# dpwe/audfprint

Hardware: NVIDIA H100
Metric: audio_seconds_fingerprinted_per_sec (higher is better)
Workload: dtype f64

## Files before the change

### audfprint_b200/csrc/afp_stft.cu

```cuda
#include <math.h>
#include <algorithm>
#include "afp_fft.cuh"
#include "afp_internal.cuh"
#include "afp_tma.cuh"

namespace {

constexpr int FT = AFP_FRAMES_PER_TILE;
constexpr int XS = 17;
constexpr int XF = 16 * XS;
constexpr int K1_THREADS = 256;
constexpr int LOGTAB = 64;
constexpr int LOGCOPIES = 8;

__device__ __forceinline__ int64_t reflect_index(int64_t j, int64_t n) {
  if (n == 1) return 0;
  const int64_t period = 2 * (n - 1);
  int64_t r = j % period;
  if (r < 0) r += period;
  return r < n ? r : period - r;
}

__device__ __forceinline__ double int_to_double(int x) {
  return __hiloint2double(0x43380000 + (x >> 31), x) - 6755399441055744.0;
}

__device__ __noinline__ double half_log_quarter_slow(double v) { return 0.5 * log(0.25 * v); }
__device__ __forceinline__ bool is_special(double v) {
  return (unsigned)(__double2hiint(v) - 0x00100000) >= 0x7fe00000u;
}

__constant__ double k1_log_c64[8] = {0.5 / 7.0, -0.5 / 6.0, 0.5 / 5.0, -0.5 / 4.0,
                                     0.5 / 3.0, -0.5 / 2.0, 0.5,       0.34657359027997264};

__device__ __forceinline__ double half_log_quarter(double v, const double2* s_logtab_lane) {
  const int hi = __double2hiint(v);
  const int lo = __double2loint(v);
  const double m = __hiloint2double((hi & 0x000fffff) | 0x3ff00000, lo);
  const double2 ct = s_logtab_lane[((hi >> 14) & (LOGTAB - 1)) * LOGCOPIES];
  const double r = fma(m, ct.x, -1.0);
  double p = k1_log_c64[0];
  p = fma(p, r, k1_log_c64[1]);
  p = fma(p, r, k1_log_c64[2]);
  p = fma(p, r, k1_log_c64[3]);
  p = fma(p, r, k1_log_c64[4]);
  p = fma(p, r, k1_log_c64[5]);
  p = fma(p, r, k1_log_c64[6]);
  const double ed = int_to_double((hi >> 20) - 1025);
  return fma(ed, k1_log_c64[7], ct.y) + p * r;
}

template <typename PcmT> struct PcmTraits;
template <> struct PcmTraits<int16_t> {
  static constexpr int NBUF = 2;
};
template <> struct PcmTraits<float> {
  static constexpr int NBUF = 1;
};

template <typename R> struct K1Traits;

template <> struct K1Traits<double> {
  using R2 = double2;
  static constexpr int MIN_CTAS = 2;
  static constexpr int LOGTAB_N = LOGTAB * LOGCOPIES;
  static constexpr int HMIN_NONE = 0x7ff00000;
  __device__ static __forceinline__ void load2(const int16_t* p, double& a, double& b) {
    const uint32_t w = *reinterpret_cast<const uint32_t*>(p);
    a = int_to_double((int)(short)(w & 0xffffu));
    b = int_to_double((int)w >> 16);
  }
  __device__ static __forceinline__ void load2(const float* p, double& a, double& b) {
    const float2 w = *reinterpret_cast<const float2*>(p);
    a = (double)w.x;
    b = (double)w.y;
  }
  __device__ static __forceinline__ int hbits(double v) { return __double2hiint(v); }
  __device__ static __forceinline__ void log_pair(double ssa, double ssb, const double2* tab, double& la,
                                                  double& lb) {
    la = half_log_quarter(ssa, tab);
    lb = half_log_quarter(ssb, tab);
    if (is_special(ssa) || is_special(ssb)) {
      la = half_log_quarter_slow(ssa);
      lb = half_log_quarter_slow(ssb);
    }
  }
  __device__ static __forceinline__ double log1(double ss, const double2* tab) {
    double lg = half_log_quarter(ss, tab);
    if (is_special(ss)) lg = half_log_quarter_slow(ss);
    return lg;
  }
  __device__ static __forceinline__ double log_lower_bound(int hmin, const double2* tab) {
    const double v_lo = __hiloint2double(hmin, 0);
    return hmin >= HMIN_NONE ? INFINITY : (hmin < 0x00100000 ? -INFINITY : half_log_quarter(v_lo, tab));
  }
};

template <> struct K1Traits<float> {
  using R2 = float2;
  static constexpr int MIN_CTAS = 3;
  static constexpr int LOGTAB_N = 0;
  static constexpr int HMIN_NONE = 0x7f800000;
  __device__ static __forceinline__ void load2(const int16_t* p, float& a, float& b) {
    const uint32_t w = *reinterpret_cast<const uint32_t*>(p);
    a = (float)(short)(w & 0xffffu);
    b = (float)((int)w >> 16);
  }
  __device__ static __forceinline__ void load2(const float* p, float& a, float& b) {
    const float2 w = *reinterpret_cast<const float2*>(p);
    a = w.x;
    b = w.y;
  }
  __device__ static __forceinline__ int hbits(float v) { return __float_as_int(v); }
  __device__ static __forceinline__ void log_pair(float ssa, float ssb, const double2*, float& la, float& lb) {
    la = 0.5f * __logf(0.25f * ssa);
    lb = 0.5f * __logf(0.25f * ssb);
  }
  __device__ static __forceinline__ float log1(float ss, const double2*) { return 0.5f * __logf(0.25f * ss); }
  __device__ static __forceinline__ double log_lower_bound(int hmin, const double2*) {
    return hmin >= HMIN_NONE ? INFINITY
           : (hmin < 0x00800000 ? -INFINITY : (double)(0.5f * __logf(0.25f * __int_as_float(hmin))) - 1e-6);
  }
};

template <typename R>
struct StftArgs {
  using R2 = typename K1Traits<R>::R2;
  const void* pcm;
  const ItemDesc* items;
  const int32_t* tile_item;
  int nitems;
  int tile_begin, tile_end;
  const R* window;
  const R2* tw256;
  const R2* w512;
  const double2* logtab;
  R* logs;
  double* nyq;
  double* tile_stats;
  double* mag;
};

struct TileInfo {
  int64_t frame0;
  int64_t src;
  int64_t j0;
  int64_t nsamples;
  int nft;
  int tma;
};

template <typename PcmT>
__device__ __forceinline__ TileInfo make_tile(const PcmT* pcm, const ItemDesc& it, int tile) {
  TileInfo ti;
  const int t0 = (tile - it.tile_base) * FT;
  ti.frame0 = it.frame_base + t0;
  ti.nft = min(FT, it.nframes - t0);
  ti.j0 = (int64_t)(t0 - 1) * AFP_N_HOP;
  ti.src = it.sample_start + ti.j0;
  ti.nsamples = it.nsamples;
  constexpr int GR = 16 / (int)sizeof(PcmT);
  const int64_t run_n = (int64_t)(ti.nft + 1) * AFP_N_HOP;
  const int64_t lo = ti.j0 < 0 ? -ti.j0 : 0;
  const int64_t hi = (ti.j0 + run_n <= it.nsamples ? run_n : it.nsamples - ti.j0) & ~(int64_t)(GR - 1);
  const bool aligned = (reinterpret_cast<uintptr_t>(pcm + ti.src) & 15) == 0;
  ti.tma = (aligned && hi > lo) ? (int)((lo << 16) | (hi - lo)) : 0;
  return ti;
}

template <typename PcmT>
__device__ __forceinline__ void stage_tile(const PcmT* pcm, const TileInfo& ti, PcmT* dst, unsigned long long* bar) {
  const int nsamp = (ti.nft + 1) * AFP_N_HOP;
  const int t_first = ti.tma >> 16, t_count = ti.tma & 0xffff;
  if (t_count && threadIdx.x == 0) bulk_copy_g2s(dst + t_first, pcm + ti.src + t_first, t_count * sizeof(PcmT), bar);
  if (t_count != nsamp) {
    const PcmT* item0 = pcm + (ti.src - ti.j0);
    for (int i = threadIdx.x; i < nsamp - t_count; i += K1_THREADS) {
      const int p = i < t_first ? i : i + t_count;
      dst[p] = item0[reflect_index(ti.j0 + p, ti.nsamples)];
    }
  }
}

template <typename R, typename PcmT>
constexpr size_t k1_smem_bytes() {
  return 512 * sizeof(R) + 2 * 256 * sizeof(typename K1Traits<R>::R2) + K1Traits<R>::LOGTAB_N * sizeof(double2) +
         2 * FT * XF * sizeof(R) + 2 * 24 * sizeof(double) + 2 * sizeof(unsigned long long) +
         PcmTraits<PcmT>::NBUF * (FT + 1) * AFP_N_HOP * sizeof(PcmT);
}

template <typename R, typename PcmT, bool WRITE_MAG>
__global__ void __launch_bounds__(K1_THREADS, K1Traits<R>::MIN_CTAS)
    afp_stft_kernel(const __grid_constant__ StftArgs<R> a) {
  using Tr = K1Traits<R>;
  using R2 = typename Tr::R2;
  constexpr int NBUF = PcmTraits<PcmT>::NBUF;
  extern __shared__ __align__(16) unsigned char smem_raw[];
  R* s_win = reinterpret_cast<R*>(smem_raw);
  R2* s_tw256 = reinterpret_cast<R2*>(s_win + 512);
  R2* s_w512 = s_tw256 + 256;
  double2* s_logtab_all = reinterpret_cast<double2*>(s_w512 + 256);
  R* s_xr = reinterpret_cast<R*>(s_logtab_all + Tr::LOGTAB_N);
  R* s_xi = s_xr + FT * XF;
  double* s_red = reinterpret_cast<double*>(s_xi + FT * XF);
  unsigned long long* s_bar = reinterpret_cast<unsigned long long*>(s_red + 2 * 24);
  PcmT* s_pcm = reinterpret_cast<PcmT*>(s_bar + 2);
  constexpr int PCM_BUF = (FT + 1) * AFP_N_HOP;
  const PcmT* pcm = reinterpret_cast<const PcmT*>(a.pcm);

  const int tid = threadIdx.x;
  if (tid == 0) mbar_init<2>(s_bar);
  for (int i = tid; i < 512; i += K1_THREADS) s_win[i] = a.window[i];
  for (int i = tid; i < 256; i += K1_THREADS) {
    s_tw256[i] = a.tw256[i];
    s_w512[i] = a.w512[i];
  }
  if constexpr (Tr::LOGTAB_N > 0)
    for (int i = tid; i < Tr::LOGTAB_N; i += K1_THREADS) s_logtab_all[i] = a.logtab[i];
  __syncthreads();

  const int g = tid >> 4;
  const int r = tid & 15;
  const int lane = tid & 31;
  const double2* s_logtab = s_logtab_all + (lane & (LOGCOPIES - 1));
  const int src_lane = (lane & 16) | ((16 - r) & 15);
  uint32_t phases = 0u;

  int tile = a.tile_begin + blockIdx.x;
  if (tile >= a.tile_end) return;
  const int G = gridDim.x;
  TileInfo cur = make_tile(pcm, a.items[a.tile_item[tile]], tile);
  TileInfo nxt = cur;
  if (tile + G < a.tile_end) nxt = make_tile(pcm, a.items[a.tile_item[tile + G]], tile + G);
  int item_nn = (tile + 2 * G < a.tile_end) ? a.tile_item[tile + 2 * G] : 0;
  stage_tile(pcm, cur, s_pcm, s_bar);
  int buf = 0;
  int red = 0;

  for (; tile < a.tile_end; tile += G) {
    const int next = tile + G;
    if (NBUF == 2 && next < a.tile_end) stage_tile(pcm, nxt, s_pcm + (buf ^ 1) * PCM_BUF, s_bar + (buf ^ 1));
    ItemDesc desc_nn = a.items[item_nn];
    const int item_n3 = (tile + 3 * G < a.tile_end) ? a.tile_item[tile + 3 * G] : 0;
    if (cur.tma & 0xffff) {
      mbar_wait(s_bar + buf, (phases >> buf) & 1u);
      phases ^= 1u << buf;
    }
    if ((cur.tma & 0xffff) != (cur.nft + 1) * AFP_N_HOP) __syncthreads();

    const bool active = g < cur.nft;
    const int64_t frame = cur.frame0 + g;
    R vmax = 0, vsum = 0;
    int hmin = Tr::HMIN_NONE;
    R zr[16], zi[16];
    if (active) {
      const PcmT* fr = s_pcm + buf * PCM_BUF + g * AFP_N_HOP;
#pragma unroll
      for (int q = 0; q < 16; ++q) {
        const int i0 = 2 * (16 * q + r);
        const R2 w = *reinterpret_cast<const R2*>(s_win + i0);
        R x0, x1;
        Tr::load2(fr + i0, x0, x1);
        zr[q] = x0 * w.x;
        zi[q] = x1 * w.y;
      }
      afp_fft16(zr, zi);
      R* xr = s_xr + g * XF;
      R* xi = s_xi + g * XF;
#pragma unroll
      for (int p = 0; p < 16; ++p) {
        const R2 w = s_tw256[p * 16 + r];
        xr[p * XS + r] = zr[p] * w.x - zi[p] * w.y;
        xi[p * XS + r] = zr[p] * w.y + zi[p] * w.x;
      }
    }
    __syncwarp();
    if (active) {
      const R* xr = s_xr + g * XF + r * XS;
      const R* xi = s_xi + g * XF + r * XS;
#pragma unroll
      for (int q = 0; q < 16; ++q) {
        zr[q] = xr[q];
        zi[q] = xi[q];
      }
      afp_fft16(zr, zi);
    }
    {
      R* out = a.logs + frame * AFP_NBINS;
#pragma unroll
      for (int s = 0; s < 8; ++s) {
        R c = __shfl_sync(0xffffffffu, zr[15 - s], src_lane);
        R d = __shfl_sync(0xffffffffu, zi[15 - s], src_lane);
        if (r == 0) {
          c = zr[(16 - s) & 15];
          d = zi[(16 - s) & 15];
        }
        if (active) {
          const int k = r + 16 * s;
          const R2 w = s_w512[k];
          const R er = zr[s] + c, ei = zi[s] - d, orr = zi[s] + d, oi = c - zr[s];
          const R pr = w.x * orr - w.y * oi, pi = w.x * oi + w.y * orr;
          const R ar = er + pr, ai = ei + pi, br = er - pr, bi = ei - pi;
          const R ssa = ar * ar + ai * ai;
          const R ssb = br * br + bi * bi;
          R la, lb;
          Tr::log_pair(ssa, ssb, s_logtab, la, lb);
          out[k] = la;
          if (k != 0) out[256 - k] = lb; else a.nyq[frame] = lb;
          if (WRITE_MAG) {
            a.mag[frame * 257 + k] = sqrt(R(0.25) * ssa);
            a.mag[frame * 257 + 256 - k] = sqrt(R(0.25) * ssb);
          }
          vmax = fmax(vmax, fmax(ssa, ssb));
          hmin = min(hmin, min(Tr::hbits(ssa), Tr::hbits(ssb)));
          vsum += la + lb;
        }
      }
      if (active && r == 0) {
        const R2 w = s_w512[128];
        const R er = R(2) * zr[8], orr = R(2) * zi[8];
        const R ar = er + w.x * orr, ai = w.y * orr;
        const R ss = ar * ar + ai * ai;
        const R lg = Tr::log1(ss, s_logtab);
        out[128] = lg;
        if (WRITE_MAG) a.mag[frame * 257 + 128] = sqrt(R(0.25) * ss);
        vmax = fmax(vmax, ss);
        hmin = min(hmin, Tr::hbits(ss));
        vsum += lg;
      }
    }
    hmin = __reduce_min_sync(0xffffffffu, hmin);
    const double vmin = Tr::log_lower_bound(hmin, s_logtab);
    double dmax = vmax, dsum = vsum;
#pragma unroll
    for (int o = 16; o > 0; o >>= 1) {
      dmax = fmax(dmax, __shfl_xor_sync(0xffffffffu, dmax, o));
      dsum += __shfl_xor_sync(0xffffffffu, dsum, o);
    }
    double* const s_part = s_red + 24 * (NBUF == 2 ? buf : red);
    if (lane == 0) {
      s_part[(tid >> 5) * 3 + 0] = dmax;
      s_part[(tid >> 5) * 3 + 1] = vmin;
      s_part[(tid >> 5) * 3 + 2] = dsum;
    }
    __syncthreads();
    if (tid == 0) {
      double m = 0.0, mn = INFINITY, sm = 0.0;
#pragma unroll
      for (int w = 0; w < K1_THREADS / 32; ++w) {
        m = fmax(m, s_part[w * 3 + 0]);
        mn = fmin(mn, s_part[w * 3 + 1]);
        sm += s_part[w * 3 + 2];
      }
      a.tile_stats[(size_t)tile * 3 + 0] = 0.25 * m;
      a.tile_stats[(size_t)tile * 3 + 1] = mn;
      a.tile_stats[(size_t)tile * 3 + 2] = sm;
    }
    if (NBUF == 2) buf ^= 1; else red ^= 1;
    cur = nxt;
    if (tile + 2 * G < a.tile_end) nxt = make_tile(pcm, desc_nn, tile + 2 * G);
    item_nn = item_n3;
    if (NBUF == 1 && next < a.tile_end) stage_tile(pcm, cur, s_pcm, s_bar);
  }
}

__global__ void afp_tile_table_kernel(const ItemDesc* items, int nitems, int32_t* tile_item) {
  const int i = blockIdx.x * blockDim.x + threadIdx.x;
  if (i >= nitems) return;
  const ItemDesc it = items[i];
  const int nt = (it.nframes + FT - 1) / FT;
  for (int k = 0; k < nt; ++k) tile_item[it.tile_base + k] = i;
}

__global__ void __launch_bounds__(256) afp_stats_kernel(const ItemDesc* items, int item0, int nitems,
                                                        const double* tile_stats, ItemStats* out, int phase) {
  const int lane = threadIdx.x & 31;
  const int w = blockIdx.x * (blockDim.x >> 5) + (threadIdx.x >> 5);
  if (w >= nitems) return;
  const int item = item0 + w;
  if (phase == 1 && !out[item].floored) return;
  const ItemDesc it = items[item];
  const int ntiles = (it.nframes + FT - 1) / FT;
  double m = 0.0, mn = INFINITY, sm = 0.0;
  for (int i = lane; i < ntiles; i += 32) {
    const double* ts = tile_stats + (size_t)(it.tile_base + i) * 3;
    m = fmax(m, ts[0]);
    mn = fmin(mn, ts[1]);
    sm += ts[2];
  }
#pragma unroll
  for (int o = 16; o > 0; o >>= 1) {
    m = fmax(m, __shfl_xor_sync(0xffffffffu, m, o));
    mn = fmin(mn, __shfl_xor_sync(0xffffffffu, mn, o));
    sm += __shfl_xor_sync(0xffffffffu, sm, o);
  }
  if (lane == 0) {
    const bool allzero = !(m > 0.0);
    ItemStats st;
    st.logfloor = allzero ? 0.0 : log(sqrt(m) / 1e6);
    st.mean = (allzero || it.nframes == 0) ? 0.0 : sm / ((double)it.nframes * 257.0);
    st.allzero = allzero ? 1 : 0;
    st.floored = (phase == 0 && !allzero && mn < st.logfloor) ? 1 : 0;
    out[item] = st;
  }
}

constexpr int FS_SPLIT = 8;
template <typename R>
__global__ void __launch_bounds__(256) afp_floorsum_kernel(const ItemDesc* items, int item0, const ItemStats* stats,
                                                           const R* logs, const double* nyq,
                                                           double* tile_stats) {
  __shared__ double s_part[8];
  const int item = item0 + blockIdx.x;
  const ItemStats st = stats[item];
  if (!st.floored) return;
  const ItemDesc it = items[item];
  const int ntiles = (it.nframes + FT - 1) / FT;
  for (int k = blockIdx.y; k < ntiles; k += FS_SPLIT) {
    const int t0 = k * FT, nft = min(FT, it.nframes - t0);
    const R* L = logs + (size_t)(it.frame_base + t0) * AFP_NBINS;
    double acc = 0.0;
    for (int i = threadIdx.x; i < nft * AFP_NBINS; i += 256) acc += fmax((double)L[i], st.logfloor);
    if ((int)threadIdx.x < nft) acc += fmax(nyq[it.frame_base + t0 + threadIdx.x], st.logfloor);
#pragma unroll
    for (int o = 16; o > 0; o >>= 1) acc += __shfl_xor_sync(0xffffffffu, acc, o);
    __syncthreads();
    if ((threadIdx.x & 31) == 0) s_part[threadIdx.x >> 5] = acc;
    __syncthreads();
    if (threadIdx.x == 0) {
      double t = 0.0;
      for (int w = 0; w < 8; ++w) t += s_part[w];
      tile_stats[(size_t)(it.tile_base + k) * 3 + 2] = t;
    }
  }
}

template <typename R>
__global__ void afp_sgram_kernel(const ItemDesc* items, const ItemStats* stats, const R* logs,
                                 double pole, double* out) {
  const ItemDesc it = items[blockIdx.x];
  const ItemStats st = stats[blockIdx.x];
  const int b = threadIdx.x;
  double z = 0.0;
  for (int t = 0; t < it.nframes; ++t) {
    const size_t idx = (size_t)(it.frame_base + t) * AFP_NBINS + b;
    double x = st.allzero ? 0.0 : __dsub_rn(fmax((double)logs[idx], st.logfloor), st.mean);
    const double y = __dadd_rn(z, x);
    z = __dadd_rn(-x, __dmul_rn(pole, y));
    out[idx] = y;
  }
}

}

int afp_launch_tile_table(afp_ctx* c) {
  if (c->nitems == 0) return AFP_OK;
  afp_tile_table_kernel<<<(c->nitems + 255) / 256, 256, 0, c->stream>>>(c->d_items.as<ItemDesc>(), c->nitems,
                                                                       c->d_tile_item.as<int32_t>());
  AFP_CUDA(c, cudaGetLastError());
  c->launches++;
  return AFP_OK;
}

namespace {

template <typename R, typename PcmT, bool WRITE_MAG>
cudaError_t launch_k1(const StftArgs<R>& a, int num_sms, int64_t ntiles, cudaStream_t stream) {
  constexpr size_t smem = k1_smem_bytes<R, PcmT>();
  const int nctas = (int)std::min<int64_t>(ntiles, (int64_t)num_sms * K1Traits<R>::MIN_CTAS);
  const cudaError_t e =
      cudaFuncSetAttribute(afp_stft_kernel<R, PcmT, WRITE_MAG>, cudaFuncAttributeMaxDynamicSharedMemorySize, (int)smem);
  if (e == cudaSuccess) afp_stft_kernel<R, PcmT, WRITE_MAG><<<nctas, K1_THREADS, smem, stream>>>(a);
  return e;
}

template <typename R>
cudaError_t launch_stft(afp_ctx* c, const DevBuf& window, const DevBuf& twid, const void* pcm, int dtype,
                        double* mag_out, int64_t tile0, int64_t ntiles) {
  using R2 = typename K1Traits<R>::R2;
  StftArgs<R> a;
  a.pcm = pcm;
  a.items = c->d_items.as<ItemDesc>();
  a.tile_item = c->d_tile_item.as<int32_t>();
  a.nitems = c->nitems;
  a.tile_begin = (int)tile0;
  a.tile_end = (int)(tile0 + ntiles);
  a.window = window.as<R>() + (dtype == AFP_PCM_I16 ? AFP_N_FFT : 0);
  a.tw256 = twid.as<R2>();
  a.w512 = twid.as<R2>() + 256;
  a.logtab = c->d_twid.as<double2>() + 512;
  a.logs = c->d_logs.as<R>();
  a.nyq = c->d_nyq.as<double>();
  a.tile_stats = c->d_tile_stats.as<double>();
  a.mag = mag_out;
  const int n = c->num_sms;
  if (dtype == AFP_PCM_I16)
    return mag_out ? launch_k1<R, int16_t, true>(a, n, ntiles, c->stream)
                   : launch_k1<R, int16_t, false>(a, n, ntiles, c->stream);
  return mag_out ? launch_k1<R, float, true>(a, n, ntiles, c->stream)
                 : launch_k1<R, float, false>(a, n, ntiles, c->stream);
}

}

int afp_launch_stft(afp_ctx* c, const void* pcm, int dtype, double* mag_out, int64_t tile0, int64_t ntiles) {
  if (ntiles <= 0) return AFP_OK;
  const cudaError_t e =
      c->ap.spectrogram_fp32
          ? launch_stft<float>(c, c->d_window_f, c->d_twid_f, pcm, dtype, mag_out, tile0, ntiles)
          : launch_stft<double>(c, c->d_window, c->d_twid, pcm, dtype, mag_out, tile0, ntiles);
  AFP_CUDA(c, e);
  AFP_CUDA(c, cudaGetLastError());
  c->launches++;
  return AFP_OK;
}

int afp_launch_stats(afp_ctx* c, int item0, int nitems) {
  if (nitems <= 0) return AFP_OK;
  const ItemDesc* items = c->d_items.as<ItemDesc>();
  ItemStats* st = c->d_item_stats.as<ItemStats>();
  double* ts = c->d_tile_stats.as<double>();
  afp_stats_kernel<<<(nitems + 7) / 8, 256, 0, c->stream>>>(items, item0, nitems, ts, st, 0);
  AFP_CUDA(c, cudaGetLastError());
  if (c->ap.spectrogram_fp32)
    afp_floorsum_kernel<float><<<dim3((unsigned)nitems, FS_SPLIT), 256, 0, c->stream>>>(
        items, item0, st, c->d_logs.as<float>(), c->d_nyq.as<double>(), ts);
  else
    afp_floorsum_kernel<double><<<dim3((unsigned)nitems, FS_SPLIT), 256, 0, c->stream>>>(
        items, item0, st, c->d_logs.as<double>(), c->d_nyq.as<double>(), ts);
  AFP_CUDA(c, cudaGetLastError());
  afp_stats_kernel<<<(nitems + 7) / 8, 256, 0, c->stream>>>(items, item0, nitems, ts, st, 1);
  AFP_CUDA(c, cudaGetLastError());
  c->launches += 3;
  return AFP_OK;
}

int afp_launch_sgram(afp_ctx* c, double* sgram_out) {
  if (c->nitems == 0 || c->total_frames == 0) return AFP_OK;
  if (c->ap.spectrogram_fp32)
    afp_sgram_kernel<float><<<c->nitems, AFP_NBINS, 0, c->stream>>>(
        c->d_items.as<ItemDesc>(), c->d_item_stats.as<ItemStats>(), c->d_logs.as<float>(), c->ap.hpf_pole, sgram_out);
  else
    afp_sgram_kernel<double><<<c->nitems, AFP_NBINS, 0, c->stream>>>(
        c->d_items.as<ItemDesc>(), c->d_item_stats.as<ItemStats>(), c->d_logs.as<double>(), c->ap.hpf_pole, sgram_out);
  AFP_CUDA(c, cudaGetLastError());
  c->launches++;
  return AFP_OK;
}
```

### audfprint_b200/csrc/afp_peaks.cu

```cuda
#include <math.h>
#include "afp_internal.cuh"
#include "afp_tma.cuh"

namespace {

constexpr unsigned FULL = 0xffffffffu;
constexpr int CH = 4;
constexpr int NST = 2;
constexpr int PFB = 8;

constexpr int K2_CTAS_PER_SM = 10;
constexpr size_t K2_SMEM_BUDGET = 233472 / K2_CTAS_PER_SM - 1024;
constexpr size_t k2_static_smem(size_t rsize) {
  return sizeof(double) * AFP_GAUSS_PAD + 128  + NST * CH * AFP_NBINS * rsize +
         NST * sizeof(unsigned long long);
}
static_assert(k2_static_smem(sizeof(double)) <= K2_SMEM_BUDGET,
              "K2's shared memory would fit fewer than 10 CTAs per SM: a 1024-item batch would run in two waves");

struct PeakArgs {
  const ItemDesc* items;
  const ItemStats* stats;
  int item0;
  const void* logs;
  const double* gauss;
  double a_dec, pole;
  int maxpks;
  double* fwd_val;
  uint8_t* fwd_bin;
  uint8_t* fwd_cnt;
  uint8_t* pk_bin;
  uint8_t* pk_cnt;
  int32_t* item_scols;
  int32_t* item_npeaks;
};

__device__ __forceinline__ int bin_of(int lane, int j) { return 8 * lane + j; }
__device__ __forceinline__ int lane_of(int pos) { return pos >> 3; }
__device__ __forceinline__ int reg_of(int pos) { return pos & 7; }
__device__ __forceinline__ int gidx(int k) { return k + (k >> 3); }

__device__ __forceinline__ void bump(double (&thr)[8], const double* sE, int lane, int pos, double val) {
  const int k0 = AFP_NBINS - pos + 8 * lane;
  const uint32_t e0 = smem_u32(sE + gidx(k0)), e1 = e0 + 8;
  const int split = 8 - (k0 & 7);
#pragma unroll
  for (int j = 0; j < 8; ++j) {
    double e;
    asm volatile("ld.shared.f64 %0, [%1];" : "=d"(e) : "r"((j >= split ? e1 : e0) + 8 * j) : "memory");
    const double p = __dmul_rn(val, e);
    thr[j] = p > thr[j] ? p : thr[j];
  }
}

__device__ __forceinline__ double pick(const double (&v)[8], int j) {
  double x = v[0];
#pragma unroll
  for (int i = 1; i < 8; ++i) x = (j == i) ? v[i] : x;
  return x;
}

__device__ __forceinline__ unsigned locmax_mask(const double (&s)[8], int lane) {
  const double left = __shfl_up_sync(FULL, s[7], 1);
  const double right = __shfl_down_sync(FULL, s[0], 1);
  bool ge[9];
  ge[0] = (lane == 0) ? true : (s[0] >= left);
#pragma unroll
  for (int j = 1; j < 8; ++j) ge[j] = s[j] >= s[j - 1];
  ge[8] = (lane == 31) ? false : (right >= s[7]);
  unsigned m = 0;
#pragma unroll
  for (int j = 0; j < 8; ++j) m |= (ge[j] && !ge[j + 1]) ? (1u << j) : 0u;
  return m;
}

__device__ __forceinline__ void spread(const double (&v)[8], double (&thr)[8], const double* sE, int lane) {
#pragma unroll
  for (int j = 0; j < 8; ++j) thr[j] = 0.0;
  const unsigned m = locmax_mask(v, lane);
  unsigned lanes = __ballot_sync(FULL, m != 0);
  while (lanes) {
    const int src = __ffs(lanes) - 1;
    lanes &= lanes - 1;
    unsigned mm = __shfl_sync(FULL, m, src);
    while (mm) {
      const int j = __ffs(mm) - 1;
      mm &= mm - 1;
      const double val = __shfl_sync(FULL, pick(v, j), src);
      bump(thr, sE, lane, bin_of(src, j), val);
    }
  }
}

__device__ __forceinline__ void hpf_step(const double (&l)[8], double (&z)[8], double (&s)[8], double lf,
                                         double mean, double pole) {
#pragma unroll
  for (int j = 0; j < 8; ++j) {
    const double x = __dsub_rn(fmax(l[j], lf), mean);
    const double y = __dadd_rn(z[j], x);
    z[j] = __dadd_rn(-x, __dmul_rn(pole, y));
    s[j] = y;
  }
}

template <typename R>
struct ColRing {
  R* buf;
  unsigned long long* bar;
  const R* src;
  int T;
  int lane;

  __device__ __forceinline__ void issue(int chunk) const {
    const int c0 = chunk * CH;
    const uint32_t bytes = (uint32_t)min(CH, T - c0) * AFP_NBINS * sizeof(R);
    bulk_copy_g2s(buf + (chunk % NST) * CH * AFP_NBINS, src + (size_t)c0 * AFP_NBINS, bytes, bar + (chunk % NST));
  }
  __device__ __forceinline__ void wait(int chunk) const { mbar_wait(bar + (chunk % NST), (chunk / NST) & 1); }
  __device__ __forceinline__ void read(const R* col, double (&x)[8]) const {
    if (sizeof(R) == 8) {
      const double2* p = reinterpret_cast<const double2*>(col) + 4 * lane;
#pragma unroll
      for (int i = 0; i < 4; ++i) {
        const double2 v = p[i];
        x[2 * i] = v.x;
        x[2 * i + 1] = v.y;
      }
    } else {
      const float4* p = reinterpret_cast<const float4*>(col) + 2 * lane;
      const float4 u = p[0], v = p[1];
      x[0] = u.x; x[1] = u.y; x[2] = u.z; x[3] = u.w;
      x[4] = v.x; x[5] = v.y; x[6] = v.z; x[7] = v.w;
    }
  }
  __device__ __forceinline__ void peek(int t, double (&x)[8]) const { read(src + (size_t)t * AFP_NBINS, x); }
  __device__ __forceinline__ void load(int t, double (&x)[8]) const {
    const int chunk = t / CH;
    if (t % CH == 0) wait(chunk);
    read(buf + ((chunk % NST) * CH + t % CH) * AFP_NBINS, x);
    if (t % CH == CH - 1 || t == T - 1) {
      __syncwarp();
      if (lane == 0 && (chunk + NST) * CH < T) issue(chunk + NST);
    }
  }
};

template <typename R>
__global__ void __launch_bounds__(32) afp_peaks_kernel(PeakArgs a) {
  __shared__ __align__(16) double sE[AFP_GAUSS_PAD];
  __shared__ __align__(128) R sCol[NST * CH * AFP_NBINS];
  __shared__ unsigned long long sBar[NST];
  const int lane = threadIdx.x;
  const int item = a.item0 + blockIdx.x;
  for (int k = lane; k < AFP_GAUSS_N; k += 32) sE[gidx(k)] = a.gauss[k];

  const ItemDesc it = a.items[item];
  const ItemStats st = a.stats[item];
  const int T = it.nframes;
  const int64_t base = it.frame_base;
  const int maxpks = a.maxpks;
  if (T == 0 || st.allzero) {
    for (int t = lane; t < T; t += 32) a.pk_cnt[base + t] = 0;
    if (lane == 0) {
      a.item_scols[item] = 0;
      a.item_npeaks[item] = 0;
    }
    return;
  }
  ColRing<R> ring{sCol, sBar, reinterpret_cast<const R*>(a.logs) + base * AFP_NBINS, T, lane};
  if (lane == 0) {
    mbar_init<NST>(sBar);
    for (int c = 0; c < NST && c * CH < T; ++c) ring.issue(c);
  }
  __syncwarp();
  const double lf = st.logfloor, mean = st.mean, pole = a.pole, a_dec = a.a_dec;

  double thr[8], z[8], s[8], sn[8], l[8];

  {
    double mx[8];
#pragma unroll
    for (int j = 0; j < 8; ++j) { z[j] = 0.0; mx[j] = -INFINITY; }
    const int n0 = min(10, T);
    for (int t = 0; t < n0; ++t) {
      ring.peek(t, l);
      hpf_step(l, z, s, lf, mean, pole);
#pragma unroll
      for (int j = 0; j < 8; ++j) mx[j] = fmax(mx[j], s[j]);
    }
    spread(mx, thr, sE, lane);
  }

#pragma unroll
  for (int j = 0; j < 8; ++j) z[j] = 0.0;
  ring.load(0, l);
  hpf_step(l, z, s, lf, mean, pole);
  unsigned lm = locmax_mask(s, lane);
  for (int t = 0; t < T; ++t) {
    unsigned lmn = 0;
    if (t + 1 < T) {
      ring.load(t + 1, l);
      hpf_step(l, z, sn, lf, mean, pole);
      lmn = locmax_mask(sn, lane);
    }
    unsigned cmask = lm;
#pragma unroll
    for (int j = 0; j < 8; ++j) cmask &= (s[j] > thr[j]) ? ~0u : ~(1u << j);
    int npk = 0;
    if (__ballot_sync(FULL, cmask != 0)) {
      while (true) {
        unsigned long long bk = 0ull;
        int bj = -1;
#pragma unroll
        for (int j = 0; j < 8; ++j) {
          const unsigned long long k = (unsigned long long)__double_as_longlong(s[j]);
          if (((cmask >> j) & 1u) && k >= bk) { bk = k; bj = j; }
        }
        const unsigned hi = (unsigned)(bk >> 32), lo = (unsigned)bk;
        const unsigned mhi = __reduce_max_sync(FULL, bj >= 0 ? hi : 0u);
        const bool v1 = bj >= 0 && hi == mhi;
        const unsigned mlo = __reduce_max_sync(FULL, v1 ? lo : 0u);
        const bool v2 = v1 && lo == mlo;
        const int pos = (int)__reduce_max_sync(FULL, v2 ? (unsigned)(bin_of(lane, bj) + 1) : 0u) - 1;
        const double val = __longlong_as_double((long long)(((unsigned long long)mhi << 32) | mlo));
        if (lane == lane_of(pos)) cmask &= ~(1u << reg_of(pos));
        bump(thr, sE, lane, pos, val);
        if (lane == 0) {
          a.fwd_val[(base + t) * maxpks + npk] = val;
          a.fwd_bin[(base + t) * maxpks + npk] = (uint8_t)pos;
        }
        ++npk;
        if (npk >= maxpks || !__ballot_sync(FULL, cmask != 0)) break;
      }
    }
    if (lane == 0) a.fwd_cnt[base + t] = (uint8_t)npk;
#pragma unroll
    for (int j = 0; j < 8; ++j) thr[j] = __dmul_rn(thr[j], a_dec);
    if (t + 1 < T) {
#pragma unroll
      for (int j = 0; j < 8; ++j) s[j] = sn[j];
      lm = lmn;
    }
  }
  __syncwarp();

  spread(s, thr, sE, lane);
  int nxt_bin = -1, nxt_alive = 0;
  int scols = 0, npeaks = 0;
  auto emit = [&](int col, int bin, int alive) {
    const unsigned am = __ballot_sync(FULL, alive != 0);
    int rank = 0;
    unsigned mm = am;
    while (mm) {
      const int src = __ffs(mm) - 1;
      mm &= mm - 1;
      const int b = __shfl_sync(FULL, bin, src);
      rank += (b < bin) ? 1 : 0;
    }
    if (alive) a.pk_bin[(base + col) * maxpks + rank] = (uint8_t)bin;
    const int c = __popc(am);
    if (lane == 0) a.pk_cnt[base + col] = (uint8_t)c;
    if (c) scols = max(scols, col + 1);
    npeaks += c;
  };
  int pc[PFB], pb[PFB];
  double pv[PFB];
  const bool slot = lane < maxpks;
  auto fetch = [&](int t, int& c, double& v, int& b) {
    c = a.fwd_cnt[base + t];
    v = slot ? a.fwd_val[(base + t) * maxpks + lane] : 0.0;
    b = slot ? (int)a.fwd_bin[(base + t) * maxpks + lane] : -1;
  };
#pragma unroll
  for (int u = 0; u < PFB; ++u)
    if (T - 1 - u >= 0) fetch(T - 1 - u, pc[u], pv[u], pb[u]);
  for (int t0 = T - 1; t0 >= 0; t0 -= PFB) {
#pragma unroll
    for (int u = 0; u < PFB; ++u) {
      const int t = t0 - u;
      if (t >= 0) {
        const int n = pc[u];
        const double my_val = pv[u];
        const int my_bin = (lane < n) ? pb[u] : -1;
        if (t - PFB >= 0) fetch(t - PFB, pc[u], pv[u], pb[u]);
        int cur_alive = 0;
        for (int k = 0; k < n; ++k) {
          const double val = __shfl_sync(FULL, my_val, k);
          const int pos = __shfl_sync(FULL, my_bin, k);
          const bool ok = val >= pick(thr, reg_of(pos));
          if ((__ballot_sync(FULL, ok) >> lane_of(pos)) & 1u) {
            bump(thr, sE, lane, pos, val);
            if (lane == k) cur_alive = 1;
            if (nxt_alive && nxt_bin == pos) nxt_alive = 0;
          }
        }
#pragma unroll
        for (int j = 0; j < 8; ++j) thr[j] = __dmul_rn(a_dec, thr[j]);
        if (t + 1 < T) emit(t + 1, nxt_bin, nxt_alive);
        nxt_bin = my_bin;
        nxt_alive = cur_alive;
      }
    }
  }
  emit(0, nxt_bin, nxt_alive);
  if (lane == 0) {
    a.item_scols[item] = scols;
    a.item_npeaks[item] = npeaks;
  }
}

__global__ void __launch_bounds__(256) afp_peaks_compact_kernel(const ItemDesc* items, int shifts, int shift,
                                                                int maxpks, const uint8_t* pk_bin,
                                                                const uint8_t* pk_cnt, const int64_t* off,
                                                                int32_t* rows) {
  __shared__ int s_scan[256];
  __shared__ int s_run;
  const ItemDesc it = items[blockIdx.x * shifts + shift];
  const int tid = threadIdx.x;
  if (tid == 0) s_run = 0;
  __syncthreads();
  int32_t* out = rows + 2 * off[blockIdx.x];
  for (int t0 = 0; t0 < it.nframes; t0 += 256) {
    const int t = t0 + tid;
    const int c = (t < it.nframes) ? pk_cnt[it.frame_base + t] : 0;
    s_scan[tid] = c;
    __syncthreads();
    for (int o = 1; o < 256; o <<= 1) {
      const int v = (tid >= o) ? s_scan[tid - o] : 0;
      __syncthreads();
      s_scan[tid] += v;
      __syncthreads();
    }
    const int excl = s_scan[tid] - c + s_run;
    for (int i = 0; i < c; ++i) {
      out[2 * (excl + i)] = t;
      out[2 * (excl + i) + 1] = pk_bin[(it.frame_base + t) * maxpks + i];
    }
    __syncthreads();
    if (tid == 255) s_run += s_scan[255];
    __syncthreads();
  }
}

__global__ void afp_gather_npeaks_kernel(const int32_t* item_npeaks, int nfiles, int shifts, int shift,
                                         int32_t* out) {
  const int f = blockIdx.x * blockDim.x + threadIdx.x;
  if (f < nfiles) out[f] = item_npeaks[f * shifts + shift];
}

__global__ void __launch_bounds__(256) afp_spread_kernel(const double* vec, int n, const double* tab,
                                                        const double* base, double* out) {
  extern __shared__ int s_pk[];
  __shared__ int s_n;
  if (threadIdx.x == 0) s_n = 0;
  __syncthreads();
  for (int i = threadIdx.x; i < n; i += blockDim.x) {
    const bool ge = (i == 0) ? true : (vec[i] >= vec[i - 1]);
    const bool ge_next = (i == n - 1) ? false : (vec[i + 1] >= vec[i]);
    if (ge && !ge_next) s_pk[atomicAdd(&s_n, 1)] = i;
  }
  __syncthreads();
  const int np = s_n;
  for (int i = threadIdx.x; i < n; i += blockDim.x) {
    double v = base ? base[i] : 0.0;
    for (int k = 0; k < np; ++k) {
      const int p = s_pk[k];
      v = fmax(v, __dmul_rn(vec[p], tab[i + n - p]));
    }
    out[i] = v;
  }
}

}

int afp_spread_peaks_impl(afp_ctx* c, const double* vector, int32_t n, const double* table, double width,
                          const double* base, double* out) {
  const size_t nn = (size_t)n;
  AFP_CUDA(c, c->d_tmp.reserve(sizeof(double) * (5 * nn + 8)));
  double* d_vec = c->d_tmp.as<double>();
  double* d_tab = d_vec + nn;
  double* d_base = d_tab + 2 * nn + 1;
  double* d_out = d_base + nn;
  std::vector<double> tab(2 * nn + 1);
  for (size_t j = 0; j < tab.size(); ++j) {
    const double u = ((double)j - (double)n) / width;
    tab[j] = table ? table[j] : exp(-0.5 * (u * u));
  }
  AFP_CUDA(c, cudaMemcpyAsync(d_vec, vector, sizeof(double) * nn, cudaMemcpyHostToDevice, c->stream));
  AFP_CUDA(c, cudaMemcpyAsync(d_tab, tab.data(), sizeof(double) * tab.size(), cudaMemcpyHostToDevice, c->stream));
  if (base) AFP_CUDA(c, cudaMemcpyAsync(d_base, base, sizeof(double) * nn, cudaMemcpyHostToDevice, c->stream));
  const size_t smem = sizeof(int) * nn;
  if (smem > 48 * 1024)
    AFP_CUDA(c, cudaFuncSetAttribute(afp_spread_kernel, cudaFuncAttributeMaxDynamicSharedMemorySize, (int)smem));
  afp_spread_kernel<<<1, 256, smem, c->stream>>>(d_vec, n, d_tab, base ? d_base : nullptr, d_out);
  AFP_CUDA(c, cudaGetLastError());
  c->launches++;
  AFP_CUDA(c, cudaMemcpyAsync(out, d_out, sizeof(double) * nn, cudaMemcpyDeviceToHost, c->stream));
  AFP_CUDA(c, cudaStreamSynchronize(c->stream));
  return AFP_OK;
}

int afp_launch_peaks(afp_ctx* c, int item0, int nitems) {
  if (nitems <= 0) return AFP_OK;
  PeakArgs a;
  a.items = c->d_items.as<ItemDesc>();
  a.stats = c->d_item_stats.as<ItemStats>();
  a.item0 = item0;
  a.logs = c->d_logs.p;
  a.gauss = c->d_gauss.as<double>();
  a.a_dec = c->ap.a_dec;
  a.pole = c->ap.hpf_pole;
  a.maxpks = c->ap.maxpksperframe;
  a.fwd_val = c->d_fwd_val.as<double>();
  a.fwd_bin = c->d_fwd_bin.as<uint8_t>();
  a.fwd_cnt = c->d_fwd_cnt.as<uint8_t>();
  a.pk_bin = c->d_pk_bin.as<uint8_t>();
  a.pk_cnt = c->d_pk_cnt.as<uint8_t>();
  a.item_scols = c->d_item_scols.as<int32_t>();
  a.item_npeaks = c->d_item_npeaks.as<int32_t>();
  if (!c->peaks_carveout_set) {
    AFP_CUDA(c, cudaFuncSetAttribute(afp_peaks_kernel<double>, cudaFuncAttributePreferredSharedMemoryCarveout,
                                     cudaSharedmemCarveoutMaxShared));
    AFP_CUDA(c, cudaFuncSetAttribute(afp_peaks_kernel<float>, cudaFuncAttributePreferredSharedMemoryCarveout,
                                     cudaSharedmemCarveoutMaxShared));
    c->peaks_carveout_set = true;
  }
  if (c->ap.spectrogram_fp32) afp_peaks_kernel<float><<<nitems, 32, 0, c->stream>>>(a);
  else afp_peaks_kernel<double><<<nitems, 32, 0, c->stream>>>(a);
  AFP_CUDA(c, cudaGetLastError());
  c->launches++;
  return AFP_OK;
}

int afp_compact_peaks(afp_ctx* c, int shift) {
  AFP_CUDA(c, c->d_tmp.reserve(sizeof(int32_t) * (size_t)(c->nfiles + 1)));
  AFP_CUDA(c, c->d_pk_off.reserve(sizeof(int64_t) * (size_t)(c->nfiles + 1)));
  afp_gather_npeaks_kernel<<<(c->nfiles + 255) / 256, 256, 0, c->stream>>>(
      c->d_item_npeaks.as<int32_t>(), c->nfiles, c->ap.shifts, shift, c->d_tmp.as<int32_t>());
  AFP_CUDA(c, cudaGetLastError());
  c->launches++;
  int rc = afp_launch_scan_i32_to_i64(c, c->d_tmp.as<int32_t>(), c->d_pk_off.as<int64_t>(), c->nfiles);
  if (rc) return rc;
  int64_t total = 0;
  AFP_CUDA(c, cudaMemcpyAsync(&total, c->d_pk_off.as<int64_t>() + c->nfiles, sizeof(int64_t),
                              cudaMemcpyDeviceToHost, c->stream));
  AFP_CUDA(c, cudaStreamSynchronize(c->stream));
  AFP_CUDA(c, c->d_pk_rows.reserve(sizeof(int32_t) * 2 * (size_t)(total + 1)));
  if (total > 0) {
    afp_peaks_compact_kernel<<<c->nfiles, 256, 0, c->stream>>>(
        c->d_items.as<ItemDesc>(), c->ap.shifts, shift, c->ap.maxpksperframe, c->d_pk_bin.as<uint8_t>(),
        c->d_pk_cnt.as<uint8_t>(), c->d_pk_off.as<int64_t>(), c->d_pk_rows.as<int32_t>());
    AFP_CUDA(c, cudaGetLastError());
    c->launches++;
  }
  return AFP_OK;
}
```

Before: 6.693 million.

## Interleave FFT scratch as complex pairs, replace shuffles with smem mirror, batch special-case logs

Stores the STFT transpose scratch as interleaved complex pairs instead of split real and imaginary arrays, which halves the number of shared-memory instructions per element. The mirrored-bin exchange for the real-FFT post-processing now goes through shared memory instead of warp shuffles, and all of it sits inside the active branch, guarded by partial-warp syncwarp masks. The per-element special-value checks on the log are replaced by a fast path plus one fallback recompute per thread, triggered from hmin/hmax. The exponent-to-double conversion is also simplified. The risks are extra shared-memory traffic, the reworked sync masks, and registers for the ss array.

```diff
diff --git a/audfprint_b200/csrc/afp_stft.cu b/audfprint_b200/csrc/afp_stft.cu
--- a/audfprint_b200/csrc/afp_stft.cu
+++ b/audfprint_b200/csrc/afp_stft.cu
@@ -30,8 +30,8 @@
   return (unsigned)(__double2hiint(v) - 0x00100000) >= 0x7fe00000u;
 }
 
-__constant__ double k1_log_c64[8] = {0.5 / 7.0, -0.5 / 6.0, 0.5 / 5.0, -0.5 / 4.0,
-                                     0.5 / 3.0, -0.5 / 2.0, 0.5,       0.34657359027997264};
+__constant__ double k1_log_c64[9] = {0.5 / 7.0, -0.5 / 6.0, 0.5 / 5.0, -0.5 / 4.0, 0.5 / 3.0,
+                                     -0.5 / 2.0, 0.5,       0.34657359027997264, 4503599627371521.0};
 
 __device__ __forceinline__ double half_log_quarter(double v, const double2* s_logtab_lane) {
   const int hi = __double2hiint(v);
@@ -46,7 +46,7 @@
   p = fma(p, r, k1_log_c64[4]);
   p = fma(p, r, k1_log_c64[5]);
   p = fma(p, r, k1_log_c64[6]);
-  const double ed = int_to_double((hi >> 20) - 1025);
+  const double ed = __hiloint2double(0x43300000, (unsigned)hi >> 20) - k1_log_c64[8];
   return fma(ed, k1_log_c64[7], ct.y) + p * r;
 }
 
@@ -76,6 +76,11 @@
     b = (double)w.y;
   }
   __device__ static __forceinline__ int hbits(double v) { return __double2hiint(v); }
+  __device__ static __forceinline__ double log_fast(double v, const double2* tab) { return half_log_quarter(v, tab); }
+  __device__ static __forceinline__ bool any_special(int hmin, int hmax) {
+    return hmin < 0x00100000 || hmax >= 0x7ff00000;
+  }
+  __device__ static __forceinline__ double max2(double x, double y) { return x > y ? x : y; }
   __device__ static __forceinline__ void log_pair(double ssa, double ssb, const double2* tab, double& la,
                                                   double& lb) {
     la = half_log_quarter(ssa, tab);
@@ -112,6 +117,9 @@
     b = w.y;
   }
   __device__ static __forceinline__ int hbits(float v) { return __float_as_int(v); }
+  __device__ static __forceinline__ float log_fast(float v, const double2*) { return 0.5f * __logf(0.25f * v); }
+  __device__ static __forceinline__ bool any_special(int, int) { return false; }
+  __device__ static __forceinline__ float max2(float x, float y) { return fmaxf(x, y); }
   __device__ static __forceinline__ void log_pair(float ssa, float ssb, const double2*, float& la, float& lb) {
     la = 0.5f * __logf(0.25f * ssa);
     lb = 0.5f * __logf(0.25f * ssb);
@@ -185,7 +193,7 @@
 template <typename R, typename PcmT>
 constexpr size_t k1_smem_bytes() {
   return 512 * sizeof(R) + 2 * 256 * sizeof(typename K1Traits<R>::R2) + K1Traits<R>::LOGTAB_N * sizeof(double2) +
-         2 * FT * XF * sizeof(R) + 2 * 24 * sizeof(double) + 2 * sizeof(unsigned long long) +
+         FT * XF * sizeof(typename K1Traits<R>::R2) + 2 * 24 * sizeof(double) + 2 * sizeof(unsigned long long) +
          PcmTraits<PcmT>::NBUF * (FT + 1) * AFP_N_HOP * sizeof(PcmT);
 }
 
@@ -200,9 +208,8 @@
   R2* s_tw256 = reinterpret_cast<R2*>(s_win + 512);
   R2* s_w512 = s_tw256 + 256;
   double2* s_logtab_all = reinterpret_cast<double2*>(s_w512 + 256);
-  R* s_xr = reinterpret_cast<R*>(s_logtab_all + Tr::LOGTAB_N);
-  R* s_xi = s_xr + FT * XF;
-  double* s_red = reinterpret_cast<double*>(s_xi + FT * XF);
+  R2* s_xz = reinterpret_cast<R2*>(s_logtab_all + Tr::LOGTAB_N);
+  double* s_red = reinterpret_cast<double*>(s_xz + FT * XF);
   unsigned long long* s_bar = reinterpret_cast<unsigned long long*>(s_red + 2 * 24);
   PcmT* s_pcm = reinterpret_cast<PcmT*>(s_bar + 2);
   constexpr int PCM_BUF = (FT + 1) * AFP_N_HOP;
@@ -223,7 +230,6 @@
   const int r = tid & 15;
   const int lane = tid & 31;
   const double2* s_logtab = s_logtab_all + (lane & (LOGCOPIES - 1));
-  const int src_lane = (lane & 16) | ((16 - r) & 15);
   uint32_t phases = 0u;
 
   int tile = a.tile_begin + blockIdx.x;
@@ -252,8 +258,10 @@
     const int64_t frame = cur.frame0 + g;
     R vmax = 0, vsum = 0;
     int hmin = Tr::HMIN_NONE;
-    R zr[16], zi[16];
     if (active) {
+      const unsigned amask = 2 * (tid >> 5) + 1 < cur.nft ? 0xffffffffu : 0x0000ffffu;
+      R2* const xz = s_xz + g * XF;
+      R zr[16], zi[16];
       const PcmT* fr = s_pcm + buf * PCM_BUF + g * AFP_N_HOP;
 #pragma unroll
       for (int q = 0; q < 16; ++q) {
@@ -265,67 +273,78 @@
         zi[q] = x1 * w.y;
       }
       afp_fft16(zr, zi);
-      R* xr = s_xr + g * XF;
-      R* xi = s_xi + g * XF;
 #pragma unroll
       for (int p = 0; p < 16; ++p) {
         const R2 w = s_tw256[p * 16 + r];
-        xr[p * XS + r] = zr[p] * w.x - zi[p] * w.y;
-        xi[p * XS + r] = zr[p] * w.y + zi[p] * w.x;
-      }
-    }
-    __syncwarp();
-    if (active) {
-      const R* xr = s_xr + g * XF + r * XS;
-      const R* xi = s_xi + g * XF + r * XS;
+        xz[p * XS + r] = R2{zr[p] * w.x - zi[p] * w.y, zr[p] * w.y + zi[p] * w.x};
+      }
+      __syncwarp(amask);
 #pragma unroll
       for (int q = 0; q < 16; ++q) {
-        zr[q] = xr[q];
-        zi[q] = xi[q];
+        const R2 v = xz[r * XS + q];
+        zr[q] = v.x;
+        zi[q] = v.y;
       }
       afp_fft16(zr, zi);
-    }
-    {
+      __syncwarp(amask);
+#pragma unroll
+      for (int s = 8; s < 16; ++s) xz[r + 16 * s] = R2{zr[s], zi[s]};
+      if (r == 0) xz[256] = R2{zr[0], zi[0]};
+      __syncwarp(amask);
+      const R2* const zp = xz + 256 - r;
       R* out = a.logs + frame * AFP_NBINS;
+      R ss[16];
+      int hmax = 0;
 #pragma unroll
       for (int s = 0; s < 8; ++s) {
-        R c = __shfl_sync(0xffffffffu, zr[15 - s], src_lane);
-        R d = __shfl_sync(0xffffffffu, zi[15 - s], src_lane);
-        if (r == 0) {
-          c = zr[(16 - s) & 15];
-          d = zi[(16 - s) & 15];
+        const R2 p = zp[-16 * s];
+        const R c = p.x, d = p.y;
+        const int k = r + 16 * s;
+        const R2 w = s_w512[k];
+        const R er = zr[s] + c, ei = zi[s] - d, orr = zi[s] + d, oi = c - zr[s];
+        const R pr = w.x * orr - w.y * oi, pi = w.x * oi + w.y * orr;
+        const R ar = er + pr, ai = ei + pi, br = er - pr, bi = ei - pi;
+        const R ssa = ar * ar + ai * ai;
+        const R ssb = br * br + bi * bi;
+        ss[2 * s] = ssa;
+        ss[2 * s + 1] = ssb;
+        const R la = Tr::log_fast(ssa, s_logtab), lb = Tr::log_fast(ssb, s_logtab);
+        out[k] = la;
+        if (k != 0) out[256 - k] = lb; else a.nyq[frame] = lb;
+        if (WRITE_MAG) {
+          a.mag[frame * 257 + k] = sqrt(R(0.25) * ssa);
+          a.mag[frame * 257 + 256 - k] = sqrt(R(0.25) * ssb);
         }
-        if (active) {
+        vmax = Tr::max2(vmax, Tr::max2(ssa, ssb));
+        hmin = min(hmin, min(Tr::hbits(ssa), Tr::hbits(ssb)));
+        hmax = max(hmax, max(Tr::hbits(ssa), Tr::hbits(ssb)));
+        vsum += la + lb;
+      }
+      if (Tr::any_special(hmin, hmax)) {
+        vmax = 0;
+        vsum = 0;
+#pragma unroll
+        for (int s = 0; s < 8; ++s) {
           const int k = r + 16 * s;
-          const R2 w = s_w512[k];
-          const R er = zr[s] + c, ei = zi[s] - d, orr = zi[s] + d, oi = c - zr[s];
-          const R pr = w.x * orr - w.y * oi, pi = w.x * oi + w.y * orr;
-          const R ar = er + pr, ai = ei + pi, br = er - pr, bi = ei - pi;
-          const R ssa = ar * ar + ai * ai;
-          const R ssb = br * br + bi * bi;
           R la, lb;
-          Tr::log_pair(ssa, ssb, s_logtab, la, lb);
+          Tr::log_pair(ss[2 * s], ss[2 * s + 1], s_logtab, la, lb);
           out[k] = la;
           if (k != 0) out[256 - k] = lb; else a.nyq[frame] = lb;
-          if (WRITE_MAG) {
-            a.mag[frame * 257 + k] = sqrt(R(0.25) * ssa);
-            a.mag[frame * 257 + 256 - k] = sqrt(R(0.25) * ssb);
-          }
-          vmax = fmax(vmax, fmax(ssa, ssb));
-          hmin = min(hmin, min(Tr::hbits(ssa), Tr::hbits(ssb)));
+          vmax = fmax(vmax, fmax(ss[2 * s], ss[2 * s + 1]));
           vsum += la + lb;
         }
       }
-      if (active && r == 0) {
+      if (r == 0) {
         const R2 w = s_w512[128];
-        const R er = R(2) * zr[8], orr = R(2) * zi[8];
+        const R2 z = xz[128];
+        const R er = R(2) * z.x, orr = R(2) * z.y;
         const R ar = er + w.x * orr, ai = w.y * orr;
-        const R ss = ar * ar + ai * ai;
-        const R lg = Tr::log1(ss, s_logtab);
+        const R s128 = ar * ar + ai * ai;
+        const R lg = Tr::log1(s128, s_logtab);
         out[128] = lg;
-        if (WRITE_MAG) a.mag[frame * 257 + 128] = sqrt(R(0.25) * ss);
-        vmax = fmax(vmax, ss);
-        hmin = min(hmin, Tr::hbits(ss));
+        if (WRITE_MAG) a.mag[frame * 257 + 128] = sqrt(R(0.25) * s128);
+        vmax = fmax(vmax, s128);
+        hmin = min(hmin, Tr::hbits(s128));
         vsum += lg;
       }
     }
```

Result: no change. 6.738 million (median of 6 runs) (+0.7%).

## Add bin-order peak acceptance fast path and ping-pong column registers

Applied to the files above, without the earlier changes.

When a column has no more threshold-passing candidates than the per-column peak limit, the candidates are accepted in bin order in one pass, and each is ranked by value with ballots. This replaces the repeated warp argmax reductions of the greedy loop, whose one-at-a-time order also decided how the threshold was bumped. Otherwise it falls back to the old greedy loop. The time loop is also unrolled by two so the s/sn register arrays swap roles instead of being copied. Accepting in bin order rather than value order changes the threshold bumping sequence, which may change which peaks are accepted.

```diff
diff --git a/audfprint_b200/csrc/afp_peaks.cu b/audfprint_b200/csrc/afp_peaks.cu
--- a/audfprint_b200/csrc/afp_peaks.cu
+++ b/audfprint_b200/csrc/afp_peaks.cu
@@ -74,10 +74,10 @@
   return m;
 }
 
-__device__ __forceinline__ void spread(const double (&v)[8], double (&thr)[8], const double* sE, int lane) {
-#pragma unroll
-  for (int j = 0; j < 8; ++j) thr[j] = 0.0;
-  const unsigned m = locmax_mask(v, lane);
+__device__ __forceinline__ unsigned long long key_of(double v) { return (unsigned long long)__double_as_longlong(v); }
+
+template <typename F>
+__device__ __forceinline__ void for_each_marked(unsigned m, const double (&v)[8], F&& f) {
   unsigned lanes = __ballot_sync(FULL, m != 0);
   while (lanes) {
     const int src = __ffs(lanes) - 1;
@@ -86,10 +86,15 @@
     while (mm) {
       const int j = __ffs(mm) - 1;
       mm &= mm - 1;
-      const double val = __shfl_sync(FULL, pick(v, j), src);
-      bump(thr, sE, lane, bin_of(src, j), val);
-    }
-  }
+      f(bin_of(src, j), __shfl_sync(FULL, pick(v, j), src));
+    }
+  }
+}
+
+__device__ __forceinline__ void spread(const double (&v)[8], double (&thr)[8], const double* sE, int lane) {
+#pragma unroll
+  for (int j = 0; j < 8; ++j) thr[j] = 0.0;
+  for_each_marked(locmax_mask(v, lane), v, [&](int pos, double val) { bump(thr, sE, lane, pos, val); });
 }
 
 __device__ __forceinline__ void hpf_step(const double (&l)[8], double (&z)[8], double (&s)[8], double lf,
@@ -191,13 +196,8 @@
     spread(mx, thr, sE, lane);
   }
 
-#pragma unroll
-  for (int j = 0; j < 8; ++j) z[j] = 0.0;
-  ring.load(0, l);
-  hpf_step(l, z, s, lf, mean, pole);
-  unsigned lm = locmax_mask(s, lane);
-  for (int t = 0; t < T; ++t) {
-    unsigned lmn = 0;
+  static_assert(AFP_MAX_PKS <= 32, "a column's accepted candidates are ranked one per lane");
+  auto column = [&](int t, const double (&s)[8], double (&sn)[8], unsigned lm, unsigned& lmn) {
     if (t + 1 < T) {
       ring.load(t + 1, l);
       hpf_step(l, z, sn, lf, mean, pole);
@@ -206,45 +206,70 @@
     unsigned cmask = lm;
 #pragma unroll
     for (int j = 0; j < 8; ++j) cmask &= (s[j] > thr[j]) ? ~0u : ~(1u << j);
+    auto put = [&](int slot, double val, int pos) {
+      a.fwd_val[(base + t) * maxpks + slot] = val;
+      a.fwd_bin[(base + t) * maxpks + slot] = (uint8_t)pos;
+    };
     int npk = 0;
     if (__ballot_sync(FULL, cmask != 0)) {
-      while (true) {
-        unsigned long long bk = 0ull;
-        int bj = -1;
-#pragma unroll
-        for (int j = 0; j < 8; ++j) {
-          const unsigned long long k = (unsigned long long)__double_as_longlong(s[j]);
-          if (((cmask >> j) & 1u) && k >= bk) { bk = k; bj = j; }
+      if ((int)__reduce_add_sync(FULL, (unsigned)__popc(cmask)) <= maxpks) {
+        double wv = 0.0;
+        int wpos = 0, rank = 0;
+        for_each_marked(cmask, s, [&](int pos, double val) {
+          bump(thr, sE, lane, pos, val);
+          const bool below = lane < npk && key_of(val) >= key_of(wv);
+          const unsigned bm = __ballot_sync(FULL, below);
+          rank += below;
+          if (lane == npk) {
+            wv = val;
+            wpos = pos;
+            rank = npk - __popc(bm);
+          }
+          ++npk;
+        });
+        if (lane < npk) put(rank, wv, wpos);
+      } else {
+        while (true) {
+          unsigned long long bk = 0ull;
+          int bj = -1;
+#pragma unroll
+          for (int j = 0; j < 8; ++j) {
+            const unsigned long long k = key_of(s[j]);
+            if (((cmask >> j) & 1u) && k >= bk) { bk = k; bj = j; }
+          }
+          const unsigned hi = (unsigned)(bk >> 32), lo = (unsigned)bk;
+          const unsigned mhi = __reduce_max_sync(FULL, bj >= 0 ? hi : 0u);
+          const bool v1 = bj >= 0 && hi == mhi;
+          const unsigned mlo = __reduce_max_sync(FULL, v1 ? lo : 0u);
+          const bool v2 = v1 && lo == mlo;
+          const int pos = (int)__reduce_max_sync(FULL, v2 ? (unsigned)(bin_of(lane, bj) + 1) : 0u) - 1;
+          const double val = __longlong_as_double((long long)(((unsigned long long)mhi << 32) | mlo));
+          if (lane == lane_of(pos)) cmask &= ~(1u << reg_of(pos));
+          bump(thr, sE, lane, pos, val);
+          if (lane == 0) put(npk, val, pos);
+          ++npk;
+          if (npk >= maxpks || !__ballot_sync(FULL, cmask != 0)) break;
         }
-        const unsigned hi = (unsigned)(bk >> 32), lo = (unsigned)bk;
-        const unsigned mhi = __reduce_max_sync(FULL, bj >= 0 ? hi : 0u);
-        const bool v1 = bj >= 0 && hi == mhi;
-        const unsigned mlo = __reduce_max_sync(FULL, v1 ? lo : 0u);
-        const bool v2 = v1 && lo == mlo;
-        const int pos = (int)__reduce_max_sync(FULL, v2 ? (unsigned)(bin_of(lane, bj) + 1) : 0u) - 1;
-        const double val = __longlong_as_double((long long)(((unsigned long long)mhi << 32) | mlo));
-        if (lane == lane_of(pos)) cmask &= ~(1u << reg_of(pos));
-        bump(thr, sE, lane, pos, val);
-        if (lane == 0) {
-          a.fwd_val[(base + t) * maxpks + npk] = val;
-          a.fwd_bin[(base + t) * maxpks + npk] = (uint8_t)pos;
-        }
-        ++npk;
-        if (npk >= maxpks || !__ballot_sync(FULL, cmask != 0)) break;
       }
     }
     if (lane == 0) a.fwd_cnt[base + t] = (uint8_t)npk;
 #pragma unroll
     for (int j = 0; j < 8; ++j) thr[j] = __dmul_rn(thr[j], a_dec);
-    if (t + 1 < T) {
-#pragma unroll
-      for (int j = 0; j < 8; ++j) s[j] = sn[j];
-      lm = lmn;
-    }
+  };
+#pragma unroll
+  for (int j = 0; j < 8; ++j) z[j] = 0.0;
+  ring.load(0, l);
+  hpf_step(l, z, s, lf, mean, pole);
+  unsigned lm = locmax_mask(s, lane), lmn = 0;
+  for (int t = 0; t < T; t += 2) {
+    column(t, s, sn, lm, lmn);
+    if (t + 1 < T) column(t + 1, sn, s, lmn, lm);
   }
   __syncwarp();
 
-  spread(s, thr, sE, lane);
+#pragma unroll
+  for (int j = 0; j < 8; ++j) l[j] = (T & 1) ? s[j] : sn[j];
+  spread(l, thr, sE, lane);
   int nxt_bin = -1, nxt_alive = 0;
   int scols = 0, npeaks = 0;
   auto emit = [&](int col, int bin, int alive) {
```

After: 6.793 million before, 6.832 million after (median of 6 runs). No clear change (+0.6%).
